# Junacik99/opengl-ray-tracer

Measured on AMD Instinct MI355X. Metric: Mrays/sec + FPS @1920x1080, car scene (4122 shapes), 1/2/4/8 GPUs, higher is better.
Workload: dtype f32

## Files before the change

opengl-ray-tracer_amd/csrc/dispatch_plan.h:

```cpp
#ifndef RT_DISPATCH_PLAN_H
#define RT_DISPATCH_PLAN_H

#include <algorithm>
#include <cstddef>

#include "../../include/rt_api.h"

namespace rtp {

constexpr size_t kTailAutoItems = 8192;
constexpr int kHeavyAutoSlots = 2;
constexpr int kLatencyMaxSlots = 12;

struct Frame {
    int width, height, y0, stripe, period, out_rows;
    float resX, resY;
};

inline unsigned long long dispatch_pixels(const Frame& k) {
    if (k.period == k.stripe)
        return static_cast<unsigned long long>(std::max(0, std::min(k.out_rows, k.height - k.y0))) * k.width;
    unsigned long long rows = 0;
    for (long long s = 0; s * k.stripe < k.out_rows; ++s) {
        const long long base = k.y0 + s * k.period;
// ... 71 lines not shown
            hp = 32;
        }
        if (!small && in.latency) {
            const int per_cu = in.tiles / std::max(1, in.cu_count);
            hk = std::max(16, in.tiles / (per_cu <= 40 ? 25 : 200));
            hp = per_cu <= 20 ? 16 : per_cu <= 40 ? 8 : in.lanes ? 2 : 4;
        }
    }
    const bool stamps_fit =
        !in.tile_times ||
        in.tile_times_cap >= static_cast<size_t>(in.tiles) + static_cast<size_t>(std::min(hk, in.tiles)) * hp;
    const bool blocks_whole = !in.ss_fused || hp * in.ss <= 8;
    if (stamps_fit && hp > 1 && hk > 0 && !in.whole && blocks_whole) return HeavySplit{std::min(hk, in.tiles), hp};
    return HeavySplit{0, 1};
}

struct TailPlan {
    int tail_from;
    bool tail;
    int rx, regions;
};

inline TailPlan tail_plan(int setting, size_t items, int maxBounces, bool ss_fused, int width, int out_rows,
                          int tiles_x, int tiles) {
    TailPlan t;
    t.tail_from = setting != RT_TAIL_AUTO ? setting : (many_items(items) ? 2 : 0);
    t.tail = t.tail_from > 0 && t.tail_from < maxBounces && !ss_fused &&
             static_cast<unsigned long long>(width) * out_rows < (1ull << 32);
    t.rx = (tiles_x + 7) / 8;
    t.regions = t.rx * ((tiles / tiles_x + 7) / 8);
    return t;
}

enum Cost { kCostNone, kCostTime, kCostCounters };

struct AccelInstance {
    bool timed, cost, tail, mt, rec, queue, ss;
};

inline AccelInstance accel_instance(bool mt, bool tile_times, bool tail, bool latency, Cost cost, bool ss_fused) {
    const bool rec = cost != kCostNone, cnt = cost == kCostCounters;
    if (ss_fused) return AccelInstance{false, cnt, !mt && latency, mt, rec, false, true};
    if (mt) return AccelInstance{false, cnt, false, true, rec, false, false};
    if (tile_times) return AccelInstance{true, true, false, false, true, false, false};
    if (tail) return AccelInstance{false, cnt, true, false, rec, true, false};
    if (latency) return AccelInstance{false, cnt, true, false, rec, false, false};
    return AccelInstance{false, cnt, false, false, rec, false, false};
}

}

#endif
```

opengl-ray-tracer_amd/csrc/rt_device.h:

```cpp
#pragma once

#include <hip/hip_runtime.h>
#include <stdint.h>

#include "srgb_table.h"

namespace rtd {

struct GeoRec {
    int type, idx;
    float f[18];
};
static_assert(sizeof(GeoRec) == 80, "GeoRec is 5 float4");

struct PrimRec {
    float f[15];
    int st;
};
static_assert(sizeof(PrimRec) == 64, "PrimRec is 4 float4");
__device__ __forceinline__ int prim_type(const PrimRec& g) { return g.st & 3; }

struct V {
    float x, y, z;
};
// ... 27 lines not shown
    const float4* __restrict__ geo_leaf;
    const float4* __restrict__ geo_lin;
    const float4* __restrict__ mat;
    const float4* __restrict__ nodes;
    int S, N, I;
    int max_stack;
    V cam_pos, cam_front, cam_right, cam_up;
    float plane_w, plane_h;
    V light_pos, light_color;
    float resX, resY;
    int maxBounces, useBVH, useFresnel, useMT;
    int width, height, y0, stripe, period, out_rows;
    char* __restrict__ dst;
    size_t pitch;
    unsigned long long* __restrict__ stats;
    unsigned long long* __restrict__ tile_times;
    int tiles_x, tiles;
    const int* __restrict__ tile_order;
    int lane_k, lane_k_mode;
    int heavy_k, heavy_parts;
    unsigned* __restrict__ tile_cost;
    int cost_time;
    unsigned long long* __restrict__ heavy_acc;
    unsigned* __restrict__ sched_hist;
    int lane_from_depth;
    int shadow_lane_from;
    int root_ok;
    float root_lo[3], root_hi[3];
    int lane_stack;
    float4* __restrict__ tail_queue;
    int* __restrict__ tail_px;
    int* __restrict__ tail_count;
    int* __restrict__ tail_count_next;
    int tail_from;
    int tail_rx, tail_regions;
    int tail_counters;
    int tail_max_lanes;
    int rgb;
    float shadow_off;
    int ss;
};

__device__ __forceinline__ int image_row(const KParams& kp, int r) {
    return kp.y0 + r + (r / kp.stripe) * (kp.period - kp.stripe);
}

__device__ __forceinline__ Ray get_ray(const KParams& kp, float ndcX, float ndcY) {
    V p = ((kp.cam_pos + kp.cam_front) + (ndcX * kp.plane_w / 2.0f) * kp.cam_right) +
          (ndcY * kp.plane_h / 2.0f) * kp.cam_up;
    return Ray{kp.cam_pos, normalize(p - kp.cam_pos)};
}

struct Hit {
    int type;
    V p;
};

__device__ __forceinline__ Hit intersect(const GeoRec& g, const Ray& r, int use_mt) {
    Hit h{NONE, V{0.f, 0.f, 0.f}};
    const float* f = g.f;
    if (g.type == 0) {
        V c = mk(f[0], f[1], f[2]);
        V oc = r.o - c;
        float aa = dot(r.d, r.d);
        float bb = 2.0f * dot(r.d, oc);
        float cc = dot(oc, oc) - f[3] * f[3];
// ... 226 lines not shown
```

opengl-ray-tracer_amd/csrc/rt_kernels.hip:

```cpp
#include <hip/hip_runtime.h>

#include <algorithm>
#include <chrono>
#include <climits>
#include <cmath>
#include <cstdio>
#include <cstdlib>
#include <cstring>
#include <functional>
#include <limits>
#include <atomic>
#include <memory>
#include <new>
#include <thread>
#include <vector>

#include "../../include/rt_api.h"
#include "accel.h"
#include "accel_math.h"
#include "accel_pack.h"
#include "refit_plan.h"
#include "lbvh.h"
#include "rt_device.h"
#include "ao_table.h"
// ... 1408 lines not shown
    else
        packet_walk<false, COST || COUNT, COUNT, MT>(A, ray, alive, 0.f, best, unused, wc);
    if (COUNT) walk_rec(rec, 2 * depth, w0, wc, clock64() - c0);
    if (alive && best.slot < 0) {
        acc = acc + mulv(att, background(kp, bg_y()));
        alive = false;
    }
    Ray sr{mk(0.f, 0.f, 0.f), mk(0.f, 0.f, 1.f)};
    float ld = 0.f;
    if (alive) {
        const V hp = hit_point(ray, best.t);
        const V hn = shape_normal(load_prim(A.prims, best.slot), hp);
        sr = Ray{hp + hn * kp.shadow_off, normalize(kp.light_pos - hp)};
        ld = dist(kp.light_pos, hp);
    }
    bool shadow = false;
    Best dummy{0.f, 0, 0.f, -1};
    w0 = wc;
    c0 = COUNT ? clock64() : 0;
    if (depth >= shadow_from)
        lane_walk_any<true, COST || COUNT, COUNT, MT, SPLIT>(A, sr, alive, gmin(ld, 1e20f), dummy, shadow, stk, stt,
                                                             blockDim.x, cap, wc);
    else
        packet_walk<true, COST || COUNT, COUNT, MT>(A, sr, alive, gmin(ld, 1e20f), dummy, shadow, wc);
    if (COUNT) walk_rec(rec, 2 * depth + 1, w0, wc, clock64() - c0);
    if (alive) {
        const PrimRec g = load_prim(A.prims, best.slot);
        const V hp = hit_point(ray, best.t);
        alive = shade_bounce(kp, ray, hp, shape_normal(g, hp), load_mat(mat, A.prim_shape[best.slot]), shadow, acc,
                             att, 1e-3f);
    }
}

template <bool COUNT, bool COST = true, bool TAIL = false, bool MT = false, bool QUEUE = TAIL, bool SS = false,
          bool DISP = false>
__device__ void accel_tile(const AccelPtrs& A, const float4* __restrict__ mat, const KParams& kp, int tile,
                           int part, int* stk, unsigned short* stt, int cap, WalkCount& wc,
                           unsigned long long* rec, bool heavy) {
    const int lane_from = heavy && (kp.lane_k_mode & 1) ? 0 : kp.lane_from_depth;
    const int shadow_from = heavy && (kp.lane_k_mode & 2) ? 0 : kp.shadow_lane_from;
    const bool mine = part == 0 || ((threadIdx.x & 63) * kp.heavy_parts >> 6) == part - 1;
    Ray ray;
    bool alive;
    {
        const PixelCoord pc = tile_pixel(kp, tile);
        ray = primary_ray(kp, pc.x, pc.y);
        alive = pc.active && mine;
    }
    V acc = mk(0.f, 0.f, 0.f), att = mk(1.f, 1.f, 1.f);
    bool deferred = false;
    if (kp.root_ok) {
        V rlo = mk(kp.root_lo[0], kp.root_lo[1], kp.root_lo[2]), rhi = mk(kp.root_hi[0], kp.root_hi[1], kp.root_hi[2]);
        if (kp.root_ok == 2) {
            const float4 a = A.anodes[4 * static_cast<size_t>(A.N - 1)], b = A.anodes[4 * static_cast<size_t>(A.N - 1) + 1];
            rlo = mk(a.x, a.y, a.z);
            rhi = mk(b.x, b.y, b.z);
        }
        const bool in = ray_aabb(ray.o, inv_dir(ray.d), rlo, rhi);
        if (alive && !in) {
            acc = background(kp, tile_pixel(kp, tile).y);
            alive = false;
        }
    }
    for (int depth = 0; depth < kp.maxBounces; ++depth) {
        if (__ballot(alive) == 0) break;
        bounce_step<COUNT, COST, MT, TAIL>(A, mat, kp, depth, ray, alive, acc, att,
                                           [&]() { return tile_pixel(kp, tile).y; }, stk, stt, cap, wc, rec,
                                           lane_from, shadow_from);
        if (TAIL && QUEUE && depth + 1 == kp.tail_from && __popcll(__ballot(alive)) <= kp.tail_max_lanes) {
            const unsigned long long m = __ballot(alive);
            if (m) {
                const int rid = (tile / kp.tiles_x / 8) * kp.tail_rx + (tile % kp.tiles_x) / 8;
                int base = 0;
                if ((threadIdx.x & 63) == 0) base = rid * kTailRegion + atomicAdd(kp.tail_count + rid, __popcll(m));
                base = __shfl(base, 0);
                if (alive) {
                    const int lane = threadIdx.x & 63;
                    const int pos = base + __popcll(m & ((1ull << lane) - 1ull));
                    const PixelCoord pc = tile_pixel(kp, tile);
                    float4* q = kp.tail_queue + 3 * static_cast<size_t>(pos);
                    q[0] = make_float4(ray.o.x, ray.o.y, ray.o.z, acc.x);
                    q[1] = make_float4(ray.d.x, ray.d.y, ray.d.z, acc.y);
                    q[2] = make_float4(att.x, att.y, att.z, acc.z);
                    kp.tail_px[pos] = static_cast<int>(static_cast<unsigned>(pc.r) * static_cast<unsigned>(kp.width) +
                                                       static_cast<unsigned>(pc.x));
                }
            }
            deferred = alive;
            break;
        }
    }
    const PixelCoord pc = tile_pixel(kp, tile);
    if (SS) {
        for (int b = 1; b < kp.ss; b <<= 1)
            acc = acc + mk(__shfl_xor(acc.x, b), __shfl_xor(acc.y, b), __shfl_xor(acc.z, b));
        for (int b = 8; b < 8 * kp.ss; b <<= 1)
            acc = acc + mk(__shfl_xor(acc.x, b), __shfl_xor(acc.y, b), __shfl_xor(acc.z, b));
        const int lane = threadIdx.x & 63;
        const float w = 1.0f / static_cast<float>(kp.ss * kp.ss);
        if (pc.active && mine && ((lane | lane >> 3) & (kp.ss - 1)) == 0)
            store_px_ss<DISP ? kStoreDisplay : kStoreFloat>(kp, pc.r, pc.x,
                                                            make_float4(acc.x * w, acc.y * w, acc.z * w, 1.0f));
        return;
    }
    if (pc.active && mine && !deferred)
        store_px<DISP ? kStoreDisplay : kStoreFloat>(kp, pc.r, pc.x, make_float4(acc.x, acc.y, acc.z, 1.0f));
}

#ifndef RT_ACCEL_ATTR
#define RT_ACCEL_ATTR __attribute__((amdgpu_waves_per_eu(4)))
#endif
template <bool TIMED, bool COST = true, bool TAIL = false, bool MT = false, bool REC = COST, bool QUEUE = TAIL,
          bool SS = false, bool DISP = false>
__global__ __launch_bounds__(kBlock) RT_ACCEL_ATTR void k_accel(AccelPtrs A, const float4* __restrict__ mat, KParams kp) {
    extern __shared__ int lds_stack[];
    int* stk = lds_stack + threadIdx.x;
    unsigned short* stt =
        reinterpret_cast<unsigned short*>(lds_stack + static_cast<size_t>(kp.lane_stack) * blockDim.x) + threadIdx.x;
    const int lane = threadIdx.x & 63;
    int tile = blockIdx.x * (blockDim.x >> 6) + (threadIdx.x >> 6);
    const int hs = kp.heavy_k * kp.heavy_parts;
    if (tile < kp.tiles + hs - kp.heavy_k) {
        unsigned long long t0 = 0;
        if (TIMED || (REC && kp.cost_time)) t0 = wall_clock64();
        int part = 0;
        const int slot = REC ? __builtin_amdgcn_readfirstlane(tile) : tile;
        if (kp.tile_order) {
            if (tile < hs) {
                part = tile % kp.heavy_parts + 1;
                tile = kp.tile_order[tile / kp.heavy_parts];
            } else {
                tile = kp.tile_order[tile - hs + kp.heavy_k];
            }
        }
        if (REC) {
            tile = __builtin_amdgcn_readfirstlane(tile);
            part = __builtin_amdgcn_readfirstlane(part);
        }
        WalkCount wc{0u, 0u, 0u, 0u};
        unsigned long long* rec =
            TIMED ? kp.tile_times + kTileRec * static_cast<size_t>(part > 0 ? kp.tiles + slot : tile) : nullptr;
        accel_tile<TIMED, COST, TAIL, MT, QUEUE, SS, DISP>(A, mat, kp, tile, part, stk, stt, kp.lane_stack, wc, rec,
                                                           slot < kp.lane_k);
        if (TIMED) {
            const unsigned long long t1 = wall_clock64();
            unsigned long long sn = wc.nodes, st = wc.tests, mn = wc.nodes, mt = wc.tests;
            for (int off = 32; off > 0; off >>= 1) {
                sn += __shfl_xor(sn, off);
                st += __shfl_xor(st, off);
                mn = max(mn, __shfl_xor(mn, off));
                mt = max(mt, __shfl_xor(mt, off));
            }
            const unsigned long long wn = wave_sum(wc.wnodes), wt = wave_sum(wc.wtests);
            if (lane == 0) {
                unsigned long long* o = rec;
                o[22] = wt;
                o[23] = wn;
                o[0] = t0;
                o[1] = t1;
                o[2] = sn;
                o[3] = st;
                o[4] = mn;
                o[5] = mt;
            }
        }
        if (REC && kp.tile_cost) {
            const unsigned long long work = !COST || kp.cost_time
                                                ? (wall_clock64() - t0) >> 2
                                                : wave_sum(static_cast<unsigned long long>(wc.nodes) + wc.tests);
            unsigned wk = static_cast<unsigned>(work < 0xffffffffull ? work : 0xffffffffull);
            bool rec = part == 0;
            if (part > 0 && lane == 0) {
                const int hk = slot / kp.heavy_parts;
                const unsigned long long old =
                    atomicAdd(&kp.heavy_acc[hk], (1ull << 56) | static_cast<unsigned long long>(wk));
                if (static_cast<int>(old >> 56) == kp.heavy_parts - 1) {
                    const unsigned long long sum = (old & ((1ull << 56) - 1)) + wk;
                    wk = static_cast<unsigned>(sum < 0xffffffffull ? sum : 0xffffffffull);
                    rec = true;
                }
            }
            if (lane == 0 && rec) {
                kp.tile_cost[tile] = wk;
                atomicAdd(&kp.sched_hist[(tile / kOrderThreads) * kOrderBuckets + work_bucket(wk)], 1u);
            }
        }
    }
}

#define RT_ACCEL_INSTANCES(X)                                                                    \
    X(false, false, false, false, false, false, false) X(false, false, false, false, false, false, true) \
    X(false, false, false, false, true, false, false) X(false, false, false, false, true, false, true)   \
    X(false, false, false, true, false, false, false) X(false, false, false, true, false, false, true)   \
    X(false, false, false, true, true, false, false) X(false, false, false, true, true, false, true)     \
    X(false, false, true, false, false, false, false) X(false, false, true, false, false, false, true)   \
    X(false, false, true, false, false, true, false) X(false, false, true, false, true, false, false)    \
    X(false, false, true, false, true, false, true) X(false, false, true, false, true, true, false)      \
    X(false, true, false, false, true, false, false) X(false, true, false, false, true, false, true)     \
    X(false, true, false, true, true, false, false) X(false, true, false, true, true, false, true)       \
    X(false, true, true, false, true, false, false) X(false, true, true, false, true, false, true)       \
    X(false, true, true, false, true, true, false) X(true, true, false, false, true, false, false)
using AccelFn = void (*)(AccelPtrs, const float4*, KParams);
struct AccelEntry {
    rtp::AccelInstance args;
    AccelFn plain, display;
};
#define RT_ACCEL_ENTRY(...) {{__VA_ARGS__}, k_accel<__VA_ARGS__>, k_accel<__VA_ARGS__, true>},
const AccelEntry kAccelTable[] = {RT_ACCEL_INSTANCES(RT_ACCEL_ENTRY)};
#undef RT_ACCEL_ENTRY

AccelFn accel_kernel(const rtp::AccelInstance& a, bool display) {
    for (const AccelEntry& e : kAccelTable) {
        const rtp::AccelInstance& b = e.args;
        if (a.timed == b.timed && a.cost == b.cost && a.tail == b.tail && a.mt == b.mt && a.rec == b.rec &&
            a.queue == b.queue && a.ss == b.ss)
            return display ? e.display : e.plain;
    }
    return nullptr;
}

__device__ __forceinline__ int wave_sum_int(int v) {
    for (int off = 32; off > 0; off >>= 1) v += __shfl_xor(v, off);
    return v;
}

__global__ __launch_bounds__(kBlock) RT_ACCEL_ATTR void k_accel_tail(AccelPtrs A, const float4* __restrict__ mat,
                                                                      KParams kp) {
    extern __shared__ int lds_stack[];
    int* stk = lds_stack + threadIdx.x;
    unsigned short* stt =
        reinterpret_cast<unsigned short*>(lds_stack + static_cast<size_t>(kp.lane_stack) * blockDim.x) + threadIdx.x;
    const int lane = threadIdx.x & 63;
    int total = 0;
    for (int b = 0; b < kp.tail_regions; b += 64) {
        const int cnt = b + lane < kp.tail_regions ? kp.tail_count[b + lane] : 0;
        total += wave_sum_int((cnt + 63) >> 6);
    }
    const int chunk = blockIdx.x * (blockDim.x >> 6) + (threadIdx.x >> 6);
    if (chunk < total) {
        int rid = 0, first = 0, n = 0, acc0 = 0;
        for (int b = 0; b < kp.tail_regions; b += 64) {
            const int cnt = b + lane < kp.tail_regions ? kp.tail_count[b + lane] : 0;
            const int ch = (cnt + 63) >> 6;
            int incl = ch;
            for (int off = 1; off < 64; off <<= 1) {
                const int y = __shfl_up(incl, off);
                if (lane >= off) incl += y;
            }
            const unsigned long long hit = __ballot(acc0 + incl > chunk && acc0 + incl - ch <= chunk && ch > 0);
            if (hit) {
                const int l = __builtin_ctzll(hit);
                rid = b + l;
                first = __shfl(acc0 + incl - ch, l);
                n = __shfl(cnt, l);
                break;
            }
            acc0 += __shfl(incl, 63);
        }
        const int k = (chunk - first) * 64 + lane;
        bool alive = k < n;
        const int i = rid * kTailRegion + k;
        Ray ray{mk(0.f, 0.f, 0.f), mk(0.f, 0.f, 1.f)};
        V acc = mk(0.f, 0.f, 0.f), att = mk(1.f, 1.f, 1.f);
        int r = 0, x = 0;
        if (alive) {
            const float4* q = kp.tail_queue + 3 * static_cast<size_t>(i);
            const float4 q0 = q[0], q1 = q[1], q2 = q[2];
            const unsigned px = static_cast<unsigned>(kp.tail_px[i]);
            ray = Ray{mk(q0.x, q0.y, q0.z), mk(q1.x, q1.y, q1.z)};
            acc = mk(q0.w, q1.w, q2.w);
            att = mk(q2.x, q2.y, q2.z);
            r = static_cast<int>(px / static_cast<unsigned>(kp.width));
            x = static_cast<int>(px - static_cast<unsigned>(r) * static_cast<unsigned>(kp.width));
        }
        const bool have = alive;
        WalkCount wc{0u, 0u, 0u, 0u};
        for (int depth = kp.tail_from; depth < kp.maxBounces; ++depth) {
            if (__ballot(alive) == 0) break;
            bounce_step<false, false, false, true>(A, mat, kp, depth, ray, alive, acc, att,
                                                   [&]() { return image_row(kp, r); }, stk, stt, kp.lane_stack, wc,
                                                   nullptr, kp.lane_from_depth, kp.shadow_lane_from);
        }
        if (have) store_px(kp, r, x, make_float4(acc.x, acc.y, acc.z, 1.0f));
    }
    if (blockIdx.x == 0)
        for (int b = threadIdx.x; b < kp.tail_counters; b += blockDim.x) kp.tail_count_next[b] = 0;
}


struct TraceArgs {
    const float4* __restrict__ rays;
    const int2* __restrict__ xy;
    float4* __restrict__ hits;
    int n;
};

__device__ __forceinline__ Ray trace_ray(const TraceArgs& q, const KParams& kp, int i, float& lim) {
    if (q.xy) {
        const int2 p = q.xy[i];
        lim = INFINITY;
        return primary_ray(kp, p.x, p.y);
    }
    const float4 a = q.rays[2 * static_cast<size_t>(i)], b = q.rays[2 * static_cast<size_t>(i) + 1];
    lim = a.w;
    return Ray{mk(a.x, a.y, a.z), mk(b.x, b.y, b.z)};
}

__device__ __forceinline__ void store_hit(const TraceArgs& q, int i, int shape, float d, bool occluded) {
    q.hits[i] = make_float4(__int_as_float(shape), d, __int_as_float(occluded ? 1 : 0), 0.0f);
}

template <int MODE, bool MT>
__global__ __launch_bounds__(kBlock) RT_ACCEL_ATTR void k_trace(AccelPtrs A, TraceArgs q, KParams kp) {
    extern __shared__ int lds_stack[];
    int* stk = lds_stack + threadIdx.x;
    unsigned short* stt =
        reinterpret_cast<unsigned short*>(lds_stack + static_cast<size_t>(kp.lane_stack) * blockDim.x) + threadIdx.x;
    const int i = blockIdx.x * blockDim.x + threadIdx.x;
    const bool active = i < q.n;
// ... 1302 lines not shown
    rt_ctx* ad_from = nullptr;
    unsigned long long* stats_dev = nullptr;
    int cu_count = 256;
    int lane_from_depth = -1;
    int cone_cull = 1;
    int split_max = kSplitMax, split_g = kSplitGroup;
    int heavy_k = kHeavyTiles, heavy_parts = kHeavyParts;
    int lane_k = -1, lane_k_mode = 2;
    int cost_time = -1;
    int latency_mode = 0;
    int* tile_order = nullptr;
    int tile_order_n = 0;
    int schedule = RT_SCHED_COST;
    unsigned* sched_cost = nullptr;
    unsigned long long* heavy_acc = nullptr;
    size_t heavy_acc_cap = 0;
    int* sched_order = nullptr;
    unsigned* sched_sets = nullptr;
    int sched_parity = 0;
    int sched_cap = 0, sched_valid = 0;
    int sched_period = 16, sched_frame = 0;
    int cost_dilate = 0;
    int moving_period = 1, moving_dilate = 1, moving_split = 0;
    FlatCamera sched_cam{};
    bool have_sched_cam = false;
    bool moving = false;
    unsigned* dil_cost = nullptr;
    size_t dil_cap = 0;
    int tail_from = RT_TAIL_AUTO;
    float4* tail_queue = nullptr;
    size_t tail_cap = 0;
    int* tail_counts = nullptr;
    int tail_regions_cap = 0;
    int tail_max_lanes = 64;
    int shadow_walk_override = -1;
    int tail_parity = 0;
    int lane_stack_override = 0;
    unsigned long long* tile_times = nullptr;
    size_t tile_times_cap = 0;
    std::vector<int> anim_ids;
    std::vector<int> refit_ids;
    std::vector<int> refit_of;
    std::vector<int> anim_cls;
    std::vector<FlatShape> anim_base;
    std::vector<int> upd_ids;
    std::vector<char> upd_mark;
    std::vector<std::pair<int, FlatShape>> upd_base;
    bool nodes_dirty = false;
    bool nodes_rebuild = false;
    bool bounds_rebuild = false;
    int updates_flushed = 0;
    int refit_mode = -1;
    long long direct_reads = 0, n_direct_slot_reads = 0;
    long long dirty_sum = 0;
    long long last_flush_bytes = 0;
    int refit_compactions = 0;
    int dirty_max = 0;
    int* anim_maps = nullptr;
    size_t anim_maps_cap = 0;
    AnimMaps anim{};
    static constexpr int kAnimRing = 3;
    void* anim_pinned[kAnimRing] = {nullptr, nullptr, nullptr};
    void* anim_pinned_dev[kAnimRing] = {nullptr, nullptr, nullptr};
    size_t anim_pinned_cap[kAnimRing] = {0, 0, 0};
    hipEvent_t anim_copied[kAnimRing] = {nullptr, nullptr, nullptr};
    size_t report_at[kAnimRing] = {0, 0, 0};
// ... 812 lines not shown
        if (rtx::create_ctx(&sub, c->device, c->stream) != RT_OK) return nullptr;
        stale = true;
    }
    return sub;
}

void inherit(rt_ctx* b, const rt_ctx* c) {
    b->cam = c->cam;
    b->light = c->light;
    b->have_cam = b->have_light = true;
    b->params = c->params;
    b->kernel = RT_KERNEL_ACCEL;
    b->lane_from_depth = c->lane_from_depth;
    b->cone_cull = c->cone_cull;
    b->split_max = c->split_max;
    b->split_g = c->split_g;
    b->heavy_k = c->heavy_k;
    b->heavy_parts = c->heavy_parts;
    b->lane_k = c->lane_k;
    b->lane_k_mode = c->lane_k_mode;
    b->cost_time = c->cost_time;
    b->latency_mode = c->latency_mode;
    b->schedule = c->schedule;
    b->sched_period = c->sched_period;
    b->cost_dilate = c->cost_dilate;
    b->moving_period = c->moving_period;
    b->moving_dilate = c->moving_dilate;
    b->moving_split = c->moving_split;
    b->frame_event = c->frame_event;
    b->refit_mode = c->refit_mode;
    b->async_rebuild = c->async_rebuild;
    b->tail_from = c->tail_from;
    b->tail_max_lanes = c->tail_max_lanes;
    b->shadow_walk_override = c->shadow_walk_override;
    b->tree_mode = c->tree_mode;
    b->scene_stack = c->scene_stack;
    b->lane_stack_override = c->lane_stack_override;
    b->ss_general = c->ss_general;
    b->adaptive = c->adaptive;
    b->convert_pass = c->convert_pass;
}

int walk_from(const rt_ctx* c) {
    if (c->lane_from_depth >= 0) return c->lane_from_depth;
    return c->accel.mt && c->N < kMtPacketMaxNodes ? kMtWalkFrom : 1;
}

bool sub_usable(const rt_ctx* b, const KParams& kp) {
    const float cmag = std::max({std::fabs(kp.cam_pos.x), std::fabs(kp.cam_pos.y), std::fabs(kp.cam_pos.z)});
    return b->accel_ok && cmag <= b->accel.origin_lim;
}

rt_ctx* brute_ctx(rt_ctx* c, const KParams& kp) {
    if (!c->brute_accel || kp.useBVH || c->S <= 0 ||
        (c->kernel != RT_KERNEL_AUTO && c->kernel != RT_KERNEL_ACCEL))
        return nullptr;
    rt_ctx* b = sub_ctx(c, c->brute, c->brute_stale);
    if (!b) return nullptr;
    if (c->brute_stale) {
        FlatNode leaf;
        std::memset(&leaf, 0, sizeof leaf);
        const float inf = std::numeric_limits<float>::infinity();
        leaf.boundsMin = rt_vec3{-inf, -inf, -inf};
        leaf.boundsMax = rt_vec3{inf, inf, inf};
        leaf.leftChild = leaf.rightChild = -1;
        leaf.startShapeIdx = 0;
// ... 197 lines not shown
        c->sched_parity = 0;
        c->sched_cap = cap;
    }
    k2.sched_hist = c->sched_sets + c->sched_parity * sched_set_words(c->sched_cap);
    const bool have = c->sched_valid == k2.tiles;
    if (have) k2.tile_order = c->sched_order;
    if (!have || c->sched_frame % period == 0) {
        k2.tile_cost = c->sched_cost;
        c->sched_frame = 0;
    }
    ++c->sched_frame;
    return RT_OK;
}

int heavy_acc_setup(rt_ctx* c, KParams& k2) {
    k2.heavy_acc = nullptr;
    if (!k2.tile_cost || k2.heavy_k <= 0) return RT_OK;
    const size_t need = static_cast<size_t>(k2.heavy_k);
    if (c->heavy_acc_cap < need)
        if (const int rc = renew_buffer(c, c->heavy_acc, c->heavy_acc_cap, need, need * sizeof(unsigned long long)))
            return rc;
    HIP_TRY(hipMemsetAsync(c->heavy_acc, 0, need * sizeof(unsigned long long), c->stream));
    k2.heavy_acc = c->heavy_acc;
    return RT_OK;
}

int tail_setup(rt_ctx* c, KParams& k2, const rtp::TailPlan& t) {
    const size_t need = static_cast<size_t>(t.regions) * kTailRegion;
    if (need > c->tail_cap)
        if (const int rc = renew_buffer(c, c->tail_queue, c->tail_cap, need, need * (3 * sizeof(float4) + sizeof(int))))
            return rc;
    if (t.regions > c->tail_regions_cap)
        if (const int rc = renew_buffer(c, c->tail_counts, c->tail_regions_cap, t.regions,
                                        2 * static_cast<size_t>(t.regions) * sizeof(int), true))
            return rc;
    k2.tail_queue = c->tail_queue;
    k2.tail_px = reinterpret_cast<int*>(c->tail_queue + 3 * c->tail_cap);
    k2.tail_count = c->tail_counts + c->tail_parity * c->tail_regions_cap;
    k2.tail_count_next = c->tail_counts + (1 - c->tail_parity) * c->tail_regions_cap;
    k2.tail_from = t.tail_from;
    k2.tail_rx = t.rx;
    k2.tail_regions = t.regions;
    k2.tail_counters = c->tail_regions_cap;
    k2.tail_max_lanes = c->tail_max_lanes;
    return RT_OK;
}

int launch_cost_order(rt_ctx* c, const KParams& k2, bool latency, int dilate, TimedSpan* span) {
    if (span)
        if (const int rc = mark_end(c, *span)) return rc;
    const unsigned* set = c->sched_sets + c->sched_parity * sched_set_words(c->sched_cap);
    unsigned* next = c->sched_sets + (1 - c->sched_parity) * sched_set_words(c->sched_cap);
    const int groups = (k2.tiles + kOrderThreads - 1) / kOrderThreads;
    const unsigned* cost = c->sched_cost;
    if (latency && c->frame_event) {
        if (!c->frame_ev && hipEventCreateWithFlags(&c->frame_ev, hipEventDisableTiming) != hipSuccess)
            return RT_ERR_DEVICE;
        HIP_TRY(hipEventRecord(c->frame_ev, c->stream));
        c->frame_ev_set = true;
    }
    if (dilate > 0) {
        const size_t need = static_cast<size_t>(k2.tiles) + static_cast<size_t>(groups) * kOrderBuckets;
        if (c->dil_cap < need)
            if (const int rc = renew_buffer(c, c->dil_cost, c->dil_cap, need, need * sizeof(unsigned))) return rc;
        hipLaunchKernelGGL(k_cost_dilate, dim3(groups), dim3(kOrderThreads), 0, c->stream, c->sched_cost,
                           k2.tiles, k2.tiles_x, dilate, c->dil_cost, c->dil_cost + k2.tiles);
        cost = c->dil_cost;
        set = c->dil_cost + k2.tiles;
// ... 32 lines not shown
    const size_t items = c->accel.st.item_ref.size();
    k2.shadow_lane_from = c->shadow_walk_override >= 0 ? c->shadow_walk_override
                          : (rtp::many_items(items) && k2.lane_from_depth <= 1 ? 0 : k2.lane_from_depth);
    k2.lane_stack = lane_stack_entries(c);
    const bool lanes = std::min(k2.lane_from_depth, k2.shadow_lane_from) < k2.maxBounces;
    const bool ordered = k2.tile_order && k2.tile_order == c->sched_order;
    if (ordered) {
        const rtp::LaneSlots ls = rtp::lane_k_slots(c->lane_k, c->lane_k_mode, lanes, k2.tiles);
        if (ls.k > 0) {
            k2.lane_k = ls.k;
            k2.lane_k_mode = ls.mode;
        }
    }
    const size_t lds = lanes || k2.lane_k > 0 ? lane_stack_lds(k2) : 0;
    if (ordered) {
        const bool whole = k2.tile_cost && c->cost_time != 0 && !c->tile_times && latency &&
                           !(c->moving && c->moving_split);
        const rtp::HeavySplit hs = rtp::heavy_split(rtp::HeavyIn{
            k2.tiles, c->cu_count, latency, lanes, c->heavy_k, c->heavy_parts, c->tile_times != nullptr,
            c->tile_times_cap, whole, sp.ss_fused, k2.ss});
        k2.heavy_k = hs.k;
        k2.heavy_parts = hs.parts;
    }
    k2.cost_time = c->cost_time != 0 ? 1 : 0;
    if (const int rc = heavy_acc_setup(c, k2)) return rc;
    const AccelPtrs A = accel_ptrs(c);
    k2.tail_queue = nullptr;
    const rtp::TailPlan tp = rtp::tail_plan(c->tail_from, items, k2.maxBounces, sp.ss_fused, k2.width, k2.out_rows,
                                            k2.tiles_x, k2.tiles);
    if (tp.tail)
        if (const int rc = tail_setup(c, k2, tp)) return rc;
    const rtp::Cost cost = !k2.tile_cost ? rtp::kCostNone : k2.cost_time ? rtp::kCostTime : rtp::kCostCounters;
    const rtp::AccelInstance inst =
        rtp::accel_instance(c->accel.mt, c->tile_times != nullptr, tp.tail, latency, cost, sp.ss_fused);
    if (!inst.queue) k2.tail_queue = nullptr;
    const AccelFn kfn = accel_kernel(inst, k2.rgb >= RT_FORMAT_RGBA8);
    if (!kfn) return RT_ERR_INVALID;
    const int blocks = k2.tiles + k2.heavy_k * (k2.heavy_parts - 1);
    hipLaunchKernelGGL(kfn, dim3(blocks), dim3(64), lds, c->stream, A, c->mat, k2);
    if (inst.queue) {
        const int tgrid = tp.regions * (kTailRegion / 64);
        hipLaunchKernelGGL(k_accel_tail, dim3(tgrid), dim3(64), lane_stack_lds(k2), c->stream, A, c->mat, k2);
        c->tail_parity = 1 - c->tail_parity;
    }
    if (sp.filter) launch_box_filter(c, kin);
    if (sp.ad_fast) {
        KParams smp = kin;
        smp.lane_stack = k2.lane_stack;
        launch_adaptive(c, A, kout, smp);
    }
    return k2.tile_cost ? launch_cost_order(c, k2, latency, dilate, span) : RT_OK;
}

int launch(rt_ctx* c, const KParams& kin, bool stats) {
    c->frame_ev_set = false;
    c->ad_ran = false;
    if (const int rc = flush_updates(c)) return rc;
    if (kin.out_rows == 0) return RT_OK;
    dim3 grid((kin.width + kTileW - 1) / kTileW, (kin.out_rows + kTileH - 1) / kTileH);
    if (grid.y > 65535u) return RT_ERR_INVALID;
    int kind = c->kernel;
    const bool usable = accel_usable(c, kin);
    if (kind == RT_KERNEL_AUTO) kind = usable ? RT_KERNEL_ACCEL : RT_KERNEL_PACKET;
    if (kind == RT_KERNEL_ACCEL && !usable) kind = RT_KERNEL_PACKET;
    const rtp::Samples sp =
        rtp::samples_plan(stats, kin.ss, kind == RT_KERNEL_ACCEL, c->tile_times != nullptr, c->ss_general,
                          c->adaptive >= 0.0f, c->convert_pass, kin.rgb >= RT_FORMAT_RGBA8);
    KParams kout = kin;
    if (sp.adaptive) {
        set_frame(kout, rtp::output_frame(frame_of(kin), kin.ss));
        kout.ss = 1;
    }
    KParams kp = sp.ad_fast ? kout : kin;
    if (sp.adaptive) {
        if (!c->ad_count && hipMalloc(&c->ad_count, 4 * sizeof(unsigned)) != hipSuccess) return RT_ERR_NO_MEMORY;
// ... 462 lines not shown
    if (!c || !c->have_scene || c->N <= 0) return false;
    std::memcpy(lo, c->root_lo, sizeof c->root_lo);
    std::memcpy(hi, c->root_hi, sizeof c->root_hi);
    return true;
}

extern "C" {

int rt_destroy(rt_ctx* c) {
    if (!c) return RT_ERR_INVALID;
    hipSetDevice(c->device);
    if (c->stream) sync_stream(c);
    if (c->brute) rt_destroy(c->brute);
    c->brute = nullptr;
    if (c->mtc) rt_destroy(c->mtc);
    c->mtc = nullptr;
    free_scene(c);
    hipFree(c->staging_shapes);
    hipFree(c->staging_nodes);
    hipFree(c->staging_idx);
    hipFree(c->img);
    hipFree(c->ss_buf);
    hipFree(c->ad_list);
    hipFree(c->ad_count);
    hipFree(c->stats_dev);
    hipFree(c->trace_in);
    hipFree(c->trace_hits);
    hipFree(c->gbuf_stage);
    hipFree(c->ao_stage);
    hipFree(c->shade_in);
    hipFree(c->shade_out);
    hipFree(c->tail_queue);
    hipFree(c->tail_counts);
    hipFree(c->tile_times);
    hipFree(c->tile_order);
    hipFree(c->sched_cost);
    hipFree(c->dil_cost);
    hipFree(c->heavy_acc);
    hipFree(c->sched_order);
    hipFree(c->sched_sets);
    hipFree(c->anim_maps);
    hipFree(c->anim_sbox);
    for (int k = 0; k < rt_ctx::kAnimRing; ++k) {
        if (c->anim_pinned[k]) hipHostFree(c->anim_pinned[k]);
        if (c->anim_copied[k]) hipEventDestroy(c->anim_copied[k]);
    }
    for (hipEvent_t e : c->ring0) if (e) hipEventDestroy(e);
    for (hipEvent_t e : c->ring1) if (e) hipEventDestroy(e);
    if (c->sync_ev) hipEventDestroy(c->sync_ev);
    if (c->frame_ev) hipEventDestroy(c->frame_ev);
    if (c->ev0) hipEventDestroy(c->ev0);
    if (c->ev1) hipEventDestroy(c->ev1);
    if (c->own_stream && c->stream) hipStreamDestroy(c->stream);
    delete c;
    return RT_OK;
}

int rt_set_stream(rt_ctx* c, void* s) {
    if (!c) return RT_ERR_INVALID;
    if (set_dev(c) != RT_OK) return RT_ERR_DEVICE;
    if (const int rc = record_mark(c)) return rc;
    HIP_TRY(sync_stream(c));
    if (c->own_stream) hipStreamDestroy(c->stream);
    if (s) {
        c->stream = static_cast<hipStream_t>(s);
        c->own_stream = false;
// ... 807 lines not shown
    return RT_OK;
}

extern "C" int rt_set_walk(rt_ctx* c, int lane_from_depth) {
    if (!c || lane_from_depth < -1) return RT_ERR_INVALID;
    c->lane_from_depth = lane_from_depth;
    return RT_OK;
}

extern "C" int rt_debug_cone_cull(rt_ctx* c, int on) {
    if (!c) return RT_ERR_INVALID;
    c->cone_cull = on ? 1 : 0;
    return c->have_scene ? upload_accel(c) : RT_OK;
}

extern "C" int rt_debug_scene_stack(rt_ctx* c, int n) {
    if (!c || n < 0) return RT_ERR_INVALID;
    c->scene_stack = n;
    return RT_OK;
}

extern "C" int rt_debug_shadow_walk(rt_ctx* c, int from) {
    if (!c || from < -1) return RT_ERR_INVALID;
    c->shadow_walk_override = from;
    return RT_OK;
}

extern "C" int rt_debug_tail_lanes(rt_ctx* c, int lanes) {
    if (!c || lanes < 0 || lanes > 64) return RT_ERR_INVALID;
    c->tail_max_lanes = lanes;
    return RT_OK;
}

extern "C" int rt_set_tail(rt_ctx* c, int from_bounce) {
    if (!c || from_bounce < RT_TAIL_AUTO) return RT_ERR_INVALID;
    c->tail_from = from_bounce;
    return RT_OK;
}

extern "C" int rt_debug_sched_period(rt_ctx* c, int period) {
    if (!c || period < 1) return RT_ERR_INVALID;
    c->sched_period = period;
    c->sched_frame = 0;
    return RT_OK;
}

extern "C" int rt_debug_moving(rt_ctx* c, int period, int dilate, int split) {
    if (!c || period < 0 || dilate < 0 || dilate > 64) return RT_ERR_INVALID;
    c->moving_period = period;
    c->moving_dilate = dilate;
    c->moving_split = split ? 1 : 0;
    return RT_OK;
}

extern "C" int rt_debug_frame_event(rt_ctx* c, int on) {
    if (!c || on < 0 || on > 1) return RT_ERR_INVALID;
    c->frame_event = on;
    return RT_OK;
}

extern "C" int rt_debug_cost_dilate(rt_ctx* c, int r) {
    if (!c || r < 0 || r > 64) return RT_ERR_INVALID;
    c->cost_dilate = r;
    return RT_OK;
}

// ... 161 lines not shown
```

opengl-ray-tracer_amd/rtamd.py:

```python
from __future__ import annotations

import ctypes as C
import os
from dataclasses import dataclass

import numpy as np

HERE = os.path.dirname(os.path.abspath(__file__))
LIBDIR = os.environ.get("RTAMD_LIBDIR") or os.path.join(HERE, "lib")


def _vec(off):
    return [("x", off), ("y", off + 4), ("z", off + 8)]


MATERIAL_DTYPE = np.dtype({
    "names": ["color", "fresnelStrength", "ambientStrength", "diffuseStrength", "specularStrength", "shininess"],
    "formats": [("<f4", 3), "<f4", "<f4", "<f4", "<f4", "<i4"],
    "offsets": [0, 12, 16, 20, 24, 28],
    "itemsize": 32,
})

SHAPE_DTYPE = np.dtype({
    "names": ["type", "material", "sphereCenter", "sphereRadius", "planeNormal", "planeD",
# ... 851 lines not shown

    def debug_ao(self, form=0, waves=0):
        fn = self._lib.rt_debug_ao
        fn.argtypes = [_P, _I, _I]
        fn.restype = _I
        self._chk(fn(self._h, int(form), int(waves)), "rt_debug_ao")

    def debug_ss_general(self, on):
        fn = self._lib.rt_debug_ss_general
        fn.argtypes = [_P, _I]
        self._chk(fn(self._h, int(bool(on))), "rt_debug_ss_general")

    def debug_convert_pass(self, on):
        fn = self._lib.rt_debug_convert_pass
        fn.argtypes = [_P, _I]
        self._chk(fn(self._h, int(bool(on))), "rt_debug_convert_pass")

    def debug_convert(self, src_ptr, src_pitch, dst_ptr, pitch, width, rows, fmt):
        fn = self._lib.rt_debug_convert
        fn.argtypes = [_P, _P, C.c_size_t, _P, C.c_size_t, _I, _I, _I]
        self._chk(fn(self._h, C.c_void_p(src_ptr), src_pitch, C.c_void_p(dst_ptr), pitch, int(width), int(rows),
                     int(fmt)), "rt_debug_convert")

    def debug_shadow_walk(self, from_bounce):
        fn = self._lib.rt_debug_shadow_walk
        fn.argtypes = [_P, _I]
        self._chk(fn(self._h, int(from_bounce)), "rt_debug_shadow_walk")

    def debug_tail_lanes(self, lanes):
        fn = self._lib.rt_debug_tail_lanes
        fn.argtypes = [_P, _I]
        self._chk(fn(self._h, int(lanes)), "rt_debug_tail_lanes")

    def set_kernel_timing(self, on):
        self._chk(self._lib.rt_set_kernel_timing(self._h, int(bool(on))), "rt_set_kernel_timing")

    def set_latency_mode(self, on):
        self._chk(self._lib.rt_set_latency_mode(self._h, int(bool(on))), "rt_set_latency_mode")

    def set_schedule(self, mode):
        self._chk(self._lib.rt_set_schedule(self._h, int(mode)), "rt_set_schedule")

    def debug_scene_stack(self, n):
        fn = self._lib.rt_debug_scene_stack
        fn.argtypes = [C.c_void_p, C.c_int]
        self._chk(fn(self._h, int(n)), "rt_debug_scene_stack")

    def debug_sched_period(self, period):
        fn = self._lib.rt_debug_sched_period
        fn.argtypes = [_P, _I]
        self._chk(fn(self._h, int(period)), "rt_debug_sched_period")

    def debug_lane_stack(self, n):
        fn = self._lib.rt_debug_lane_stack
        fn.argtypes = [_P, _I]
        self._chk(fn(self._h, int(n)), "rt_debug_lane_stack")

    def debug_tile_order(self, order):
        fn = self._lib.rt_debug_tile_order
        fn.argtypes = [_P, _P, _I]
        o = np.ascontiguousarray(order if order is not None else [], np.int32)
        self._chk(fn(self._h, _ptr(o) if o.size else None, int(o.size)), "rt_debug_tile_order")

    def debug_anim_rebuilds(self):
        fn = self._lib.rt_debug_anim_rebuilds
        fn.argtypes = [_P]
# ... 296 lines not shown
```

Baseline: 22770.

## Precompute tail chunk prefix in a plan kernel and size tail grid adaptively

```diff
diff --git a/opengl-ray-tracer_amd/csrc/dispatch_plan.h b/opengl-ray-tracer_amd/csrc/dispatch_plan.h
--- a/opengl-ray-tracer_amd/csrc/dispatch_plan.h
+++ b/opengl-ray-tracer_amd/csrc/dispatch_plan.h
@@ -127,20 +127,30 @@
     return t;
 }
 
+constexpr int kTailGridMin = 1024;
+inline int tail_grid(int estimate, int upper, int forced) {
+    upper = std::max(1, upper);
+    if (forced > 0) return std::min(forced, upper);
+    const long long want = static_cast<long long>(std::max(0, estimate)) + std::max(0, estimate) / 8 + 16;
+    return static_cast<int>(std::min<long long>(upper, std::max<long long>(kTailGridMin, want)));
+}
+
 enum Cost { kCostNone, kCostTime, kCostCounters };
 
 struct AccelInstance {
     bool timed, cost, tail, mt, rec, queue, ss;
+    bool split = false;
 };
 
-inline AccelInstance accel_instance(bool mt, bool tile_times, bool tail, bool latency, Cost cost, bool ss_fused) {
+inline AccelInstance accel_instance(bool mt, bool tile_times, bool tail, bool latency, Cost cost, bool ss_fused,
+                                    bool small = false) {
     const bool rec = cost != kCostNone, cnt = cost == kCostCounters;
-    if (ss_fused) return AccelInstance{false, cnt, !mt && latency, mt, rec, false, true};
-    if (mt) return AccelInstance{false, cnt, false, true, rec, false, false};
-    if (tile_times) return AccelInstance{true, true, false, false, true, false, false};
-    if (tail) return AccelInstance{false, cnt, true, false, rec, true, false};
-    if (latency) return AccelInstance{false, cnt, true, false, rec, false, false};
-    return AccelInstance{false, cnt, false, false, rec, false, false};
+    if (ss_fused) return AccelInstance{false, cnt, !mt && latency, mt, rec, false, true, !mt && latency};
+    if (mt) return AccelInstance{false, cnt, false, true, rec, false, false, false};
+    if (tile_times) return AccelInstance{true, true, false, false, true, false, false, false};
+    if (tail) return AccelInstance{false, cnt, true, false, rec, true, false, !small || latency};
+    if (latency) return AccelInstance{false, cnt, true, false, rec, false, false, true};
+    return AccelInstance{false, cnt, false, false, rec, false, false, false};
 }
 
 }
diff --git a/opengl-ray-tracer_amd/csrc/rt_device.h b/opengl-ray-tracer_amd/csrc/rt_device.h
--- a/opengl-ray-tracer_amd/csrc/rt_device.h
+++ b/opengl-ray-tracer_amd/csrc/rt_device.h
@@ -83,6 +83,9 @@
     int* __restrict__ tail_px;
     int* __restrict__ tail_count;
     int* __restrict__ tail_count_next;
+    int* __restrict__ tail_prefix;
+    int* __restrict__ tail_coarse;
+    int* __restrict__ tail_total_host;
     int tail_from;
     int tail_rx, tail_regions;
     int tail_counters;
diff --git a/opengl-ray-tracer_amd/csrc/rt_kernels.hip b/opengl-ray-tracer_amd/csrc/rt_kernels.hip
--- a/opengl-ray-tracer_amd/csrc/rt_kernels.hip
+++ b/opengl-ray-tracer_amd/csrc/rt_kernels.hip
@@ -1464,7 +1464,7 @@
     }
 }
 
-template <bool COUNT, bool COST = true, bool TAIL = false, bool MT = false, bool QUEUE = TAIL, bool SS = false,
+template <bool COUNT, bool COST = true, bool SPLIT = false, bool MT = false, bool QUEUE = SPLIT, bool SS = false,
           bool DISP = false>
 __device__ void accel_tile(const AccelPtrs& A, const float4* __restrict__ mat, const KParams& kp, int tile,
                            int part, int* stk, unsigned short* stt, int cap, WalkCount& wc,
@@ -1496,10 +1496,10 @@
     }
     for (int depth = 0; depth < kp.maxBounces; ++depth) {
         if (__ballot(alive) == 0) break;
-        bounce_step<COUNT, COST, MT, TAIL>(A, mat, kp, depth, ray, alive, acc, att,
-                                           [&]() { return tile_pixel(kp, tile).y; }, stk, stt, cap, wc, rec,
-                                           lane_from, shadow_from);
-        if (TAIL && QUEUE && depth + 1 == kp.tail_from && __popcll(__ballot(alive)) <= kp.tail_max_lanes) {
+        bounce_step<COUNT, COST, MT, SPLIT>(A, mat, kp, depth, ray, alive, acc, att,
+                                            [&]() { return tile_pixel(kp, tile).y; }, stk, stt, cap, wc, rec,
+                                            lane_from, shadow_from);
+        if (QUEUE && depth + 1 == kp.tail_from && __popcll(__ballot(alive)) <= kp.tail_max_lanes) {
             const unsigned long long m = __ballot(alive);
             if (m) {
                 const int rid = (tile / kp.tiles_x / 8) * kp.tail_rx + (tile % kp.tiles_x) / 8;
@@ -1542,7 +1542,7 @@
 #ifndef RT_ACCEL_ATTR
 #define RT_ACCEL_ATTR __attribute__((amdgpu_waves_per_eu(4)))
 #endif
-template <bool TIMED, bool COST = true, bool TAIL = false, bool MT = false, bool REC = COST, bool QUEUE = TAIL,
+template <bool TIMED, bool COST = true, bool SPLIT = false, bool MT = false, bool REC = COST, bool QUEUE = SPLIT,
           bool SS = false, bool DISP = false>
 __global__ __launch_bounds__(kBlock) RT_ACCEL_ATTR void k_accel(AccelPtrs A, const float4* __restrict__ mat, KParams kp) {
     extern __shared__ int lds_stack[];
@@ -1572,8 +1572,8 @@
         WalkCount wc{0u, 0u, 0u, 0u};
         unsigned long long* rec =
             TIMED ? kp.tile_times + kTileRec * static_cast<size_t>(part > 0 ? kp.tiles + slot : tile) : nullptr;
-        accel_tile<TIMED, COST, TAIL, MT, QUEUE, SS, DISP>(A, mat, kp, tile, part, stk, stt, kp.lane_stack, wc, rec,
-                                                           slot < kp.lane_k);
+        accel_tile<TIMED, COST, SPLIT, MT, QUEUE, SS, DISP>(A, mat, kp, tile, part, stk, stt, kp.lane_stack, wc, rec,
+                                                            slot < kp.lane_k);
         if (TIMED) {
             const unsigned long long t1 = wall_clock64();
             unsigned long long sn = wc.nodes, st = wc.tests, mn = wc.nodes, mt = wc.tests;
@@ -1631,13 +1631,18 @@
     X(false, true, false, false, true, false, false) X(false, true, false, false, true, false, true)     \
     X(false, true, false, true, true, false, false) X(false, true, false, true, true, false, true)       \
     X(false, true, true, false, true, false, false) X(false, true, true, false, true, false, true)       \
-    X(false, true, true, false, true, true, false) X(true, true, false, false, true, false, false)
+    X(false, true, true, false, true, true, false) X(true, true, false, false, true, false, false)     \
+    X(false, false, false, false, false, true, false) X(false, false, false, false, true, true, false)   \
+    X(false, true, false, false, true, true, false)
 using AccelFn = void (*)(AccelPtrs, const float4*, KParams);
 struct AccelEntry {
     rtp::AccelInstance args;
     AccelFn plain, display;
 };
-#define RT_ACCEL_ENTRY(...) {{__VA_ARGS__}, k_accel<__VA_ARGS__>, k_accel<__VA_ARGS__, true>},
+#define RT_ACCEL_ENTRY(TIMED, COST, SPLIT, MT, REC, QUEUE, SS) \
+    {{TIMED, COST, SPLIT || QUEUE, MT, REC, QUEUE, SS, SPLIT},   \
+     k_accel<TIMED, COST, SPLIT, MT, REC, QUEUE, SS>,            \
+     k_accel<TIMED, COST, SPLIT, MT, REC, QUEUE, SS, true>},
 const AccelEntry kAccelTable[] = {RT_ACCEL_INSTANCES(RT_ACCEL_ENTRY)};
 #undef RT_ACCEL_ENTRY
 
@@ -1645,17 +1650,44 @@
     for (const AccelEntry& e : kAccelTable) {
         const rtp::AccelInstance& b = e.args;
         if (a.timed == b.timed && a.cost == b.cost && a.tail == b.tail && a.mt == b.mt && a.rec == b.rec &&
-            a.queue == b.queue && a.ss == b.ss)
+            a.queue == b.queue && a.ss == b.ss && a.split == b.split)
             return display ? e.display : e.plain;
     }
     return nullptr;
 }
 
-__device__ __forceinline__ int wave_sum_int(int v) {
-    for (int off = 32; off > 0; off >>= 1) v += __shfl_xor(v, off);
-    return v;
-}
-
+__global__ __launch_bounds__(64) void k_tail_plan(KParams kp) {
+    const int lane = threadIdx.x & 63;
+    int acc0 = 0;
+    for (int b = 0; b < kp.tail_regions; b += 64) {
+        const int cnt = b + lane < kp.tail_regions ? kp.tail_count[b + lane] : 0;
+        const int ch = (cnt + 63) >> 6;
+        int incl = ch;
+        for (int off = 1; off < 64; off <<= 1) {
+            const int y = __shfl_up(incl, off);
+            if (lane >= off) incl += y;
+        }
+        if (b + lane < kp.tail_regions) kp.tail_prefix[b + lane] = acc0 + incl - ch;
+        if (lane == 0) kp.tail_coarse[b >> 6] = acc0;
+        acc0 += __shfl(incl, 63);
+    }
+    if (lane == 0) {
+        kp.tail_prefix[kp.tail_regions] = acc0;
+        *kp.tail_total_host = acc0;
+    }
+    for (int b = lane; b < kp.tail_counters; b += 64) kp.tail_count_next[b] = 0;
+}
+
+__device__ __forceinline__ int tail_find(const int* __restrict__ pre, int n, int c) {
+    const int lane = threadIdx.x & 63;
+    for (int b = 0; b < n; b += 64) {
+        const unsigned long long le = __ballot(b + lane < n && pre[b + lane] <= c);
+        if (~le) return b + __popcll(le) - 1;
+    }
+    return n - 1;
+}
+
+template <bool SPLIT>
 __global__ __launch_bounds__(kBlock) RT_ACCEL_ATTR void k_accel_tail(AccelPtrs A, const float4* __restrict__ mat,
                                                                       KParams kp) {
     extern __shared__ int lds_stack[];
@@ -1663,32 +1695,13 @@
     unsigned short* stt =
         reinterpret_cast<unsigned short*>(lds_stack + static_cast<size_t>(kp.lane_stack) * blockDim.x) + threadIdx.x;
     const int lane = threadIdx.x & 63;
-    int total = 0;
-    for (int b = 0; b < kp.tail_regions; b += 64) {
-        const int cnt = b + lane < kp.tail_regions ? kp.tail_count[b + lane] : 0;
-        total += wave_sum_int((cnt + 63) >> 6);
-    }
-    const int chunk = blockIdx.x * (blockDim.x >> 6) + (threadIdx.x >> 6);
-    if (chunk < total) {
-        int rid = 0, first = 0, n = 0, acc0 = 0;
-        for (int b = 0; b < kp.tail_regions; b += 64) {
-            const int cnt = b + lane < kp.tail_regions ? kp.tail_count[b + lane] : 0;
-            const int ch = (cnt + 63) >> 6;
-            int incl = ch;
-            for (int off = 1; off < 64; off <<= 1) {
-                const int y = __shfl_up(incl, off);
-                if (lane >= off) incl += y;
-            }
-            const unsigned long long hit = __ballot(acc0 + incl > chunk && acc0 + incl - ch <= chunk && ch > 0);
-            if (hit) {
-                const int l = __builtin_ctzll(hit);
-                rid = b + l;
-                first = __shfl(acc0 + incl - ch, l);
-                n = __shfl(cnt, l);
-                break;
-            }
-            acc0 += __shfl(incl, 63);
-        }
+    const int total = __builtin_amdgcn_readfirstlane(kp.tail_prefix[kp.tail_regions]);
+    for (int chunk = __builtin_amdgcn_readfirstlane(blockIdx.x); chunk < total;
+         chunk = __builtin_amdgcn_readfirstlane(chunk + gridDim.x)) {
+        const int blk = tail_find(kp.tail_coarse, (kp.tail_regions + 63) >> 6, chunk);
+        const int rid = __builtin_amdgcn_readfirstlane(
+            64 * blk + tail_find(kp.tail_prefix + 64 * blk, min(64, kp.tail_regions - 64 * blk), chunk));
+        const int first = kp.tail_prefix[rid], n = kp.tail_count[rid];
         const int k = (chunk - first) * 64 + lane;
         bool alive = k < n;
         const int i = rid * kTailRegion + k;
@@ -1709,14 +1722,12 @@
         WalkCount wc{0u, 0u, 0u, 0u};
         for (int depth = kp.tail_from; depth < kp.maxBounces; ++depth) {
             if (__ballot(alive) == 0) break;
-            bounce_step<false, false, false, true>(A, mat, kp, depth, ray, alive, acc, att,
-                                                   [&]() { return image_row(kp, r); }, stk, stt, kp.lane_stack, wc,
-                                                   nullptr, kp.lane_from_depth, kp.shadow_lane_from);
+            bounce_step<false, false, false, SPLIT>(A, mat, kp, depth, ray, alive, acc, att,
+                                                    [&]() { return image_row(kp, r); }, stk, stt, kp.lane_stack, wc,
+                                                    nullptr, kp.lane_from_depth, kp.shadow_lane_from);
         }
         if (have) store_px(kp, r, x, make_float4(acc.x, acc.y, acc.z, 1.0f));
     }
-    if (blockIdx.x == 0)
-        for (int b = threadIdx.x; b < kp.tail_counters; b += blockDim.x) kp.tail_count_next[b] = 0;
 }
 
 
@@ -3085,6 +3096,10 @@
     size_t tail_cap = 0;
     int* tail_counts = nullptr;
     int tail_regions_cap = 0;
+    int* tail_total = nullptr;
+    int* tail_total_dev = nullptr;
+    int tail_grid = 0;
+    int tail_last_grid = 0;
     int tail_max_lanes = 64;
     int shadow_walk_override = -1;
     int tail_parity = 0;
@@ -3963,6 +3978,7 @@
     b->async_rebuild = c->async_rebuild;
     b->tail_from = c->tail_from;
     b->tail_max_lanes = c->tail_max_lanes;
+    b->tail_grid = c->tail_grid;
     b->shadow_walk_override = c->shadow_walk_override;
     b->tree_mode = c->tree_mode;
     b->scene_stack = c->scene_stack;
@@ -4226,8 +4242,19 @@
             return rc;
     if (t.regions > c->tail_regions_cap)
         if (const int rc = renew_buffer(c, c->tail_counts, c->tail_regions_cap, t.regions,
-                                        2 * static_cast<size_t>(t.regions) * sizeof(int), true))
+                                        (3 * static_cast<size_t>(t.regions) + 1 + (t.regions + 63) / 64) * sizeof(int),
+                                        true))
             return rc;
+    if (!c->tail_total) {
+        if (hipHostMalloc(&c->tail_total, sizeof(int), hipHostMallocMapped | hipHostMallocCoherent) != hipSuccess)
+            return RT_ERR_NO_MEMORY;
+        *c->tail_total = 0;
+        if (hipHostGetDevicePointer(reinterpret_cast<void**>(&c->tail_total_dev), c->tail_total, 0) != hipSuccess)
+            return RT_ERR_DEVICE;
+    }
+    k2.tail_prefix = c->tail_counts + 2 * static_cast<size_t>(c->tail_regions_cap);
+    k2.tail_coarse = k2.tail_prefix + c->tail_regions_cap + 1;
+    k2.tail_total_host = c->tail_total_dev;
     k2.tail_queue = c->tail_queue;
     k2.tail_px = reinterpret_cast<int*>(c->tail_queue + 3 * c->tail_cap);
     k2.tail_count = c->tail_counts + c->tail_parity * c->tail_regions_cap;
@@ -4326,15 +4353,20 @@
         if (const int rc = tail_setup(c, k2, tp)) return rc;
     const rtp::Cost cost = !k2.tile_cost ? rtp::kCostNone : k2.cost_time ? rtp::kCostTime : rtp::kCostCounters;
     const rtp::AccelInstance inst =
-        rtp::accel_instance(c->accel.mt, c->tile_times != nullptr, tp.tail, latency, cost, sp.ss_fused);
+        rtp::accel_instance(c->accel.mt, c->tile_times != nullptr, tp.tail, latency, cost, sp.ss_fused,
+                            !rtp::many_items(items));
     if (!inst.queue) k2.tail_queue = nullptr;
     const AccelFn kfn = accel_kernel(inst, k2.rgb >= RT_FORMAT_RGBA8);
     if (!kfn) return RT_ERR_INVALID;
     const int blocks = k2.tiles + k2.heavy_k * (k2.heavy_parts - 1);
     hipLaunchKernelGGL(kfn, dim3(blocks), dim3(64), lds, c->stream, A, c->mat, k2);
     if (inst.queue) {
-        const int tgrid = tp.regions * (kTailRegion / 64);
-        hipLaunchKernelGGL(k_accel_tail, dim3(tgrid), dim3(64), lane_stack_lds(k2), c->stream, A, c->mat, k2);
+        hipLaunchKernelGGL(k_tail_plan, dim3(1), dim3(64), 0, c->stream, k2);
+        const int estimate = *static_cast<volatile const int*>(c->tail_total);
+        const int tgrid = rtp::tail_grid(estimate, tp.regions * (kTailRegion / 64), c->tail_grid);
+        hipLaunchKernelGGL(inst.split ? k_accel_tail<true> : k_accel_tail<false>, dim3(tgrid), dim3(64),
+                           lane_stack_lds(k2), c->stream, A, c->mat, k2);
+        c->tail_last_grid = tgrid;
         c->tail_parity = 1 - c->tail_parity;
     }
     if (sp.filter) launch_box_filter(c, kin);
@@ -4863,6 +4895,7 @@
     hipFree(c->shade_out);
     hipFree(c->tail_queue);
     hipFree(c->tail_counts);
+    if (c->tail_total) hipHostFree(c->tail_total);
     hipFree(c->tile_times);
     hipFree(c->tile_order);
     hipFree(c->sched_cost);
@@ -5736,6 +5769,19 @@
     return RT_OK;
 }
 
+extern "C" int rt_debug_tail_grid(rt_ctx* c, int waves) {
+    if (!c || waves < 0) return RT_ERR_INVALID;
+    c->tail_grid = waves;
+    return RT_OK;
+}
+
+extern "C" int rt_debug_tail_stats(rt_ctx* c, int* out) {
+    if (!c || !out) return RT_ERR_INVALID;
+    out[0] = c->tail_last_grid;
+    out[1] = c->tail_total ? *static_cast<volatile const int*>(c->tail_total) : 0;
+    return RT_OK;
+}
+
 extern "C" int rt_set_tail(rt_ctx* c, int from_bounce) {
     if (!c || from_bounce < RT_TAIL_AUTO) return RT_ERR_INVALID;
     c->tail_from = from_bounce;
diff --git a/opengl-ray-tracer_amd/rtamd.py b/opengl-ray-tracer_amd/rtamd.py
--- a/opengl-ray-tracer_amd/rtamd.py
+++ b/opengl-ray-tracer_amd/rtamd.py
@@ -907,6 +907,18 @@
         fn.argtypes = [_P, _I]
         self._chk(fn(self._h, int(lanes)), "rt_debug_tail_lanes")
 
+    def debug_tail_grid(self, waves):
+        fn = self._lib.rt_debug_tail_grid
+        fn.argtypes = [_P, _I]
+        self._chk(fn(self._h, int(waves)), "rt_debug_tail_grid")
+
+    def debug_tail_stats(self):
+        fn = self._lib.rt_debug_tail_stats
+        out = (C.c_int * 2)()
+        fn.argtypes = [_P, C.POINTER(C.c_int)]
+        self._chk(fn(self._h, out), "rt_debug_tail_stats")
+        return int(out[0]), int(out[1])
+
     def set_kernel_timing(self, on):
         self._chk(self._lib.rt_set_kernel_timing(self._h, int(bool(on))), "rt_set_kernel_timing")
 
```

After: 22760, median of 4. About the same (-0.0%).
